# andrew-sha/CUDAFluidSimulator

Measured on AMD Instinct MI355X. Metric: particle-steps/sec (first 41 of the 100 steps of -m time), higher is better.
Workload: dtype f32

## Files before the change

### cudafluidsimulator_amd/csrc/sweeps_list.hip

```cpp
#include "sweep_common.h"

#define SL_NONE 0xFFFFFFFFu

#ifndef SL_WINDOW
#define SL_WINDOW 160
#endif
#ifndef SL_K1_THREADS
#define SL_K1_THREADS 64
#endif

#ifndef SL_K1_WAVES
#define SL_K1_WAVES 6
#endif
__device__ __forceinline__ void sl_store_quiet(const SweepArgs &A, int i, bool valid, float rho, int lane) {
    const unsigned long long calm = A.calm[(i - lane) >> 6];
    const float prs = fmaxf(0.f, SPH_GAS_CONSTANT * (rho - SPH_REST_DENSITY));
    const bool q = valid && prs == 0.f && ((calm >> lane) & 1ull);
    const unsigned long long qb = __ballot(q), vb = __ballot(valid);
    if (lane == 0) {
        reinterpret_cast<unsigned long long *>(A.quiet)[(i - lane) >> 6] = qb;
        if (A.quietAll && qb != vb) *A.quietAll = 0u;
    }
}
__device__ __forceinline__ uint32_t sl_quiet_window(const uint32_t *__restrict__ quiet, uint32_t j) {
    const uint32_t lo = quiet[j >> 5], hi = quiet[(j >> 5) + 1];
    return __builtin_amdgcn_alignbit(hi, lo, j & 31u);
}

template <bool FAST, bool SAMECUT>
__global__ __launch_bounds__(SL_K1_THREADS, SL_K1_WAVES * SL_K1_THREADS / 64)
void k_density_mask_lds(DevParams P, SweepArgs A) {
    __shared__ float4 stageAll[SL_K1_THREADS / SPH_WAVE][SW_CAP + SW_UNROLL];
    const int lane = threadIdx.x & 63, w = threadIdx.x >> 6;
    float4 *stage = stageAll[w];
    const int wv = xcd_tile(blockIdx.x, gridDim.x, A.tileChunk * (256 / SL_K1_THREADS), A.tileRotate) * (SL_K1_THREADS / SPH_WAVE) + w;
    const int i = A.i_origin + wv * SPH_WAVE + lane;
    const bool valid = i >= A.i_begin && i < A.i_end;
    const bool anyValid = __ballot(valid) != 0ull;
    float4 pi = valid ? A.pos4[i] : make_float4(0, 0, 0, 0);
    int3 c = sweep_cell(P, pi.x, pi.y, pi.z);
    int js[9], je[9];
    load_runs(P, A.cellRange, c, valid, js, je);

    int words = 0;
    uint32_t pairs = 0;
#pragma unroll
    for (int r = 0; r < 9; ++r) {
        words += (je[r] - js[r] + 31) >> 5;
        pairs += (uint32_t)(je[r] - js[r]);
    }
    const int Q = __builtin_amdgcn_readfirstlane((wave_max_i32(words) + 1) >> 1);
    const int shard = wv & (SL_POOL_SHARDS - 1);
    unsigned long long base = 0;
    if (lane == 0) base = atomicAdd(A.maskCursor + shard * SL_CURSOR_STRIDE, (unsigned long long)Q * SPH_WAVE);
    base = (unsigned long long)__builtin_amdgcn_readfirstlane((unsigned)(base >> 32)) << 32 |
           (unsigned long long)__builtin_amdgcn_readfirstlane((unsigned)base);
    const unsigned long long subCap = A.maskCapacity / SL_POOL_SHARDS;
    const bool ok = base + (unsigned long long)Q * SPH_WAVE <= subCap;
    base += (unsigned long long)shard * subCap;
    if (lane == 0 && anyValid) {
        A.maskOff[2 * (size_t)wv] = ok ? (uint32_t)base : SL_NONE;
        A.maskOff[2 * (size_t)wv + 1] = (uint32_t)Q;
        if (!ok) A.noneList[atomicAdd(A.maskCursor + 1, 1ull)] = (uint32_t)wv;
    }
    uint4 *const myq = reinterpret_cast<uint4 *>(A.maskPool) + (ok ? base : 0ull) + lane;
    if (A.pairCounter) {
        uint32_t s = wave_sum_u32(pairs);
        if (lane == 0) atomicAdd(A.pairCounter + 16 + (wv & 255) * 16, (unsigned long long)s);
    }

    if (lane < SW_UNROLL) stage[SW_CAP + lane] = make_float4(1e18f, 1e18f, 1e18f, 0.f);
    const float4 *const sent = stage + SW_CAP;
    float rho = 0.f;
    float h2v = P.h2, dcv = P.dcoef, cut2r = P.cut2, massv = SPH_MASS;
    asm volatile("" : "+v"(h2v), "+v"(dcv), "+v"(cut2r), "+v"(massv));
    uint32_t pj0 = 0, pm0 = 0;
    bool pending = false;
    int qidx = 0;
    uint32_t hcount = 0;
    auto emit = [&](uint32_t jbase, uint32_t mask) {
        if (ok && mask != 0) {
            hcount += (uint32_t)__builtin_popcount(mask);
            if (!pending) {
                pj0 = jbase;
                pm0 = mask;
                pending = true;
            } else {
                myq[(size_t)qidx * SPH_WAVE] = make_uint4(pj0, pm0, jbase, mask);
                ++qidx;
                pending = false;
            }
        }
    };
    const int rowId = c.y + c.z * P.D;
    unsigned long long todo = __ballot(valid);
    bool unify = false;
    if (todo) {
        const int row0 = __builtin_amdgcn_readlane(rowId, __ffsll((long long)todo) - 1);
        if (__ballot(valid && rowId != row0)) {
            unify = true;
#pragma unroll
            for (int r = 0; r < 9; ++r) {
                const unsigned long long mm = __ballot(valid && je[r] > js[r]);
                if (mm) {
                    const int u0 = __builtin_amdgcn_readlane(js[r], __ffsll((long long)mm) - 1);
                    const int u1 = __builtin_amdgcn_readlane(je[r], 63 - __clzll((long long)mm));
                    unify = unify && (u1 - u0) <= SW_CAP;
                }
            }
        }
    }
    struct Run {
        int jsr, len, u0, ulen;
        bool any, staged;
    };
    auto describe = [&](int r, bool act) -> Run {
        int jsr = js[0], jer = je[0];
#pragma unroll
        for (int q = 1; q < 9; ++q) {
            jsr = (r == q) ? js[q] : jsr;
            jer = (r == q) ? je[q] : jer;
        }
        Run R;
        const bool nonempty = act && jer > jsr;
        const unsigned long long mm = __ballot(nonempty);
        R.any = mm != 0;
        const int lo = mm ? __ffsll((long long)mm) - 1 : 0;
        const int hi = mm ? 63 - __clzll((long long)mm) : 0;
        R.u0 = __builtin_amdgcn_readlane(jsr, lo);
        R.ulen = R.any ? __builtin_amdgcn_readlane(jer, hi) - R.u0 : 0;
        R.staged = R.ulen <= SW_CAP;
        R.jsr = nonempty ? jsr : R.u0;
        R.len = nonempty ? jer - jsr : 0;
        return R;
    };
    while (todo) {
        const int leader = __ffsll((long long)todo) - 1;
        const int rowL = __builtin_amdgcn_readlane(rowId, leader);
        const bool act = valid && (unify || rowId == rowL);
        todo &= ~__ballot(act);
#pragma unroll 1
        for (int r = 0; r < 9; ++r) {
            const Run R = describe(r, act);
            if (R.any && R.staged) {
                for (int k = lane; k < R.ulen; k += SPH_WAVE) stage[k] = A.pos4[R.u0 + k];
                __builtin_amdgcn_fence(__ATOMIC_RELEASE, "wavefront");
                __builtin_amdgcn_wave_barrier();
            }
            if (R.any) {
                const int jsr = R.jsr, len = R.len;
                const float4 *cur = stage + (jsr - R.u0);
                const float4 *gcur = A.pos4 + jsr;
                uint32_t m = 0;
                int k = 0;
                auto trip = [&](const float4 (&pj)[SW_UNROLL]) {
#pragma unroll
                    for (int u = 0; u < SW_UNROLL; ++u) {
                        float dx = pi.x - pj[u].x;
                        float dy = pi.y - pj[u].y;
                        float dz = pi.z - pj[u].z;
                        float dist2;
                        float draw;
                        if (FAST) {
                            dist2 = __builtin_fmaf(dz, dz, __builtin_fmaf(dy, dy, dx * dx));
                            draw = h2v - dist2;
                            const float diff = fmaxf(draw, 0.f);
                            rho = __builtin_fmaf((massv * dcv) * (diff * diff), diff, rho);
                        } else {
                            dist2 = dx * dx + dy * dy + dz * dz;
                            draw = h2v - dist2;
                            float diff;
                            asm("v_max_f32_e32 %0, 0, %1" : "=v"(diff) : "v"(draw));
                            rho += massv * (dcv * diff * diff * diff);
                        }
                        if (SAMECUT) {
                            m = __builtin_amdgcn_alignbit(m, __float_as_uint(draw), 31);
                            continue;
                        }
                        asm("v_cmp_ngt_f32_e32 vcc, %1, %2\n\tv_addc_co_u32_e32 %0, vcc, %0, %0, vcc"
                            : "+v"(m)
                            : "v"(dist2), "v"(cut2r)
                            : "vcc");
                    }
#pragma unroll
                    for (int u = 0; u < SW_UNROLL; ++u) asm volatile("" ::"v"(pj[u].w));
                    if (((k + SW_UNROLL) & 31) == 0) {
                        if (SAMECUT) emit((uint32_t)(jsr + (k & ~31)), ~__builtin_bitreverse32(m));
                        else emit((uint32_t)(jsr + (k & ~31)), __builtin_bitreverse32(m));
                        m = 0;
                    }
                };
                if (R.staged) {
                    for (; __ballot(k < len); k += SW_UNROLL) {
                        float4 pj[SW_UNROLL];
#pragma unroll
                        for (int u = 0; u < SW_UNROLL; ++u) {
                            const float4 *p = (k + u < len) ? cur + k : sent;
                            pj[u] = p[u];
                        }
                        trip(pj);
                    }
                } else {
                    for (; __ballot(k < len); k += SW_UNROLL) {
                        float4 pj[SW_UNROLL];
#pragma unroll
                        for (int u = 0; u < SW_UNROLL; ++u) {
                            const bool in = k + u < len;
                            pj[u] = gcur[in ? k + u : 0];
                            pj[u].x = in ? pj[u].x : 1e18f;
                        }
                        trip(pj);
                    }
                }
                if ((k & 31) != 0) {
                    if (SAMECUT) emit((uint32_t)(jsr + (k & ~31)), (~__builtin_bitreverse32(m)) >> (32 - (k & 31)));
                    else emit((uint32_t)(jsr + (k & ~31)), __builtin_bitreverse32(m) >> (32 - (k & 31)));
                }
                __builtin_amdgcn_fence(__ATOMIC_ACQUIRE, "wavefront");
                __builtin_amdgcn_wave_barrier();
            }
        }
    }
    if (ok && valid) {
        if (pending) myq[(size_t)qidx * SPH_WAVE] = make_uint4(pj0, pm0, 0u, 0u);
        else if (qidx < Q) myq[(size_t)qidx * SPH_WAVE] = make_uint4(0u, 0u, 0u, 0u);
    }
    if (valid) {
        rho = fmaxf(rho, SPH_EPS_F);
        if (A.rhoToVel4) A.vel4[i].w = rho;
        A.pv8[2 * (size_t)i + 1].w = rho;
    }
    if (A.quiet) sl_store_quiet(A, i, valid, rho, lane);
    if (A.hitCount && valid) A.hitCount[i] = hcount;
}

#ifndef SL_SORT_SHIFT
#define SL_SORT_SHIFT 3
#endif
#define SL_DEAL_THREADS 256
#define SL_DEAL_ROWS SL_DEAL_THREADS
#define SL_DEAL_WINDOW (SL_DEAL_ROWS + SL_WINDOW - SPH_WAVE)
static_assert(SL_WINDOW >= SPH_WAVE, "the dealt sweep needs the window");

template <bool FAST, bool SLIM>
__global__ __launch_bounds__(SL_DEAL_THREADS) void k_force_dealt(DevParams P, SweepArgs A) {
    __shared__ uint32_t sortBase[128];
    __shared__ uint16_t rowOf[SL_DEAL_ROWS];
    __shared__ float4 win[2 * SL_DEAL_WINDOW];
    const int t = threadIdx.x, lane = t & 63;
    const bool second = (int)blockIdx.x >= A.nblk1;
    const int rb = second ? A.i_begin2 : A.i_begin, re = second ? A.i_end2 : A.i_end;
    const int chunk = A.tileChunk > 0 ? max(A.tileChunk * 256 / SL_DEAL_ROWS, 1) : 0;
    const int group = ((rb - A.i_origin) >> 6) / (SL_DEAL_ROWS / SPH_WAVE) +
                      xcd_tile(second ? (int)blockIdx.x - A.nblk1 : (int)blockIdx.x,
                               second ? (int)gridDim.x - A.nblk1 : A.nblk1, chunk, A.tileRotate);
    const int R0 = A.i_origin + group * SL_DEAL_ROWS;
    const unsigned long long *const quiet64 = reinterpret_cast<const unsigned long long *>(A.quiet);

    unsigned long long qw = 0ull;
    bool inPlace = false;
    if (A.quiet) {
        const int r0 = R0 + (t & ~63);
        const int lo = max(rb - r0, 0), hi = min(re - r0, 64);
        const unsigned long long vm = hi > lo ? ((hi - lo == 64 ? ~0ull : (1ull << (hi - lo)) - 1ull) << lo) : 0ull;
        if (vm) qw = quiet64[r0 >> 6];
        inPlace = __syncthreads_and((qw & vm) == vm) != 0;
    }
    if (!inPlace) {
        for (int b = t; b < 128; b += SL_DEAL_THREADS) sortBase[b] = 0u;
        __syncthreads();
        const int row = R0 + t;
        const bool counted = row >= rb && row < re && !((qw >> lane) & 1ull);
        const uint32_t bucket = min((counted ? A.hitCount[row] : 0u) >> SL_SORT_SHIFT, 127u);
        const uint32_t slot = atomicAdd(&sortBase[bucket], 1u);
        __syncthreads();
        if (t < SPH_WAVE) {
            const uint32_t a = sortBase[2 * t], b = sortBase[2 * t + 1];
            uint32_t incl = a + b;
#pragma unroll
            for (int off = 1; off < SPH_WAVE; off <<= 1) {
                const uint32_t up = __shfl_up(incl, off);
                incl += t >= off ? up : 0u;
            }
            const uint32_t excl = incl - (a + b);
            sortBase[2 * t] = excl;
            sortBase[2 * t + 1] = excl + a;
        }
        __syncthreads();
        rowOf[sortBase[bucket] + slot] = (uint16_t)t;
    }

    const bool allQuiet = A.quietAll && __builtin_amdgcn_readfirstlane(*A.quietAll) != 0u &&
                          (!A.quietHalo || __builtin_amdgcn_readfirstlane(*A.quietHalo) != 0u);
    const int w0 = max(R0 - (SL_WINDOW - SPH_WAVE) / 2, 0);
    int wlen = max(min(SL_DEAL_WINDOW, A.n_all - w0), 0);
    {
        bool wanted = !allQuiet && wlen > 0;
        if (wanted && A.quiet) {
            const int k0 = w0 >> 6, k1 = (w0 + wlen - 1) >> 6;
            wanted = k0 + t <= k1 && quiet64[k0 + t] != ~0ull;
        }
        if (__syncthreads_or(wanted)) {
            for (int k = t; k < 2 * wlen; k += SL_DEAL_THREADS) win[k] = A.pv8[2 * (size_t)w0 + k];
            __syncthreads();
        } else {
            wlen = 0;
        }
    }

    {
        const int i = R0 + (inPlace ? t : (int)rowOf[t]);
        const bool inRange = i >= rb && i < re;
        const int iSafe = inRange ? i : rb;
        float4 pi = A.pv8[2 * (size_t)iSafe];
        const float4 vi = A.pv8[2 * (size_t)iSafe + 1];
        const float prs_i = fmaxf(0.f, SPH_GAS_CONSTANT * (vi.w - SPH_REST_DENSITY));
        const int rel = iSafe - A.i_origin;
        const uint32_t baseq = inRange ? A.maskOff[2 * (size_t)(rel >> 6)] : SL_NONE;
        const int Q = inRange ? (int)A.maskOff[2 * (size_t)(rel >> 6) + 1] : 0;
        const bool valid = inRange && baseq != SL_NONE;
        ForceAcc F = {0.f, 0.f, 0.f};
        if (!allQuiet) {
            const uint4 *const sbase = reinterpret_cast<const uint4 *>(A.maskPool);
            const uint32_t send = valid ? baseq + (uint32_t)Q * SPH_WAVE : 0u;
            uint32_t sidx = valid ? baseq + (uint32_t)(rel & 63) : 0u;
            uint32_t m = 0, mq[2] = {0u, 0u};
            int jb = 0, jq[2] = {0, 0};
            bool live = true;
            const bool qi = A.quiet && valid && ((A.quiet[i >> 5] >> (i & 31)) & 1u);
            auto fetch = [&]() {
                while (sidx < send) {
                    uint4 q = sbase[sidx];
                    sidx = (q.w == 0u) ? send : sidx + SPH_WAVE;
                    if (qi) {
                        q.y &= ~sl_quiet_window(A.quiet, q.x);
                        q.w &= ~sl_quiet_window(A.quiet, q.z);
                    }
                    if (q.y == 0u) {
                        q.x = q.z;
                        q.y = q.w;
                        q.w = 0u;
                    }
                    jq[0] = (int)q.x;
                    mq[0] = q.y;
                    jq[1] = (int)q.z;
                    mq[1] = q.w;
                    if (q.y != 0u) break;
                }
            };
            fetch();
            if (__ballot(mq[0] != 0u)) {
                auto pop = [&]() -> int {
                    if (m == 0) {
                        m = mq[0];
                        jb = jq[0];
                        mq[0] = mq[1];
                        jq[0] = jq[1];
                        mq[1] = 0;
                        if (mq[0] == 0) fetch();
                    }
                    live = (m | mq[0]) != 0;
                    const bool has = m != 0;
                    const int b = has ? __builtin_ctz(m) : 0;
                    m &= m - 1u;
                    return has ? jb + b : iSafe;
                };
                auto body = [&](const float4 &pj, const float4 &vj) {
                    if (FAST) force_pair_fast(P, pi.x, pi.y, pi.z, vi.x, vi.y, vi.z, prs_i, pj, vj, F);
                    else force_pair<SLIM>(P, pi.x, pi.y, pi.z, vi.x, vi.y, vi.z, prs_i, pj, vj, F);
                };
#define SD_UNDEF4(q) asm volatile("" : "=v"(q.x), "=v"(q.y), "=v"(q.z), "=v"(q.w));
#define SD_FETCH(j, p, v)                                                      \
    SD_UNDEF4(p)                                                               \
    SD_UNDEF4(v)                                                               \
    if ((unsigned)((j)-w0) >= (unsigned)wlen) {                                \
        p = A.pv8[2 * (size_t)(j)];                                            \
        v = A.pv8[2 * (size_t)(j) + 1];                                        \
    }
#define SD_USE(j, p, v)                                                        \
    if ((unsigned)((j)-w0) < (unsigned)wlen) {                                 \
        p = win[2 * ((j)-w0)];                                                 \
        v = win[2 * ((j)-w0) + 1];                                             \
    }                                                                          \
    body(p, v);
                float4 p0 = make_float4(0, 0, 0, 0), v0 = p0, p1 = p0, v1 = p0;
                int j0 = pop();
                SD_FETCH(j0, p0, v0)
                int j1 = pop();
                SD_FETCH(j1, p1, v1)
                for (;;) {
                    SD_USE(j0, p0, v0)
                    if (!__ballot(live)) { SD_USE(j1, p1, v1) break; }
                    j0 = pop();
                    SD_FETCH(j0, p0, v0)
                    SD_USE(j1, p1, v1)
                    if (!__ballot(live)) { SD_USE(j0, p0, v0) break; }
                    j1 = pop();
                    SD_FETCH(j1, p1, v1)
                }
#undef SD_FETCH
#undef SD_USE
#undef SD_UNDEF4
            }
        }
        if (valid) {
            float vx = vi.x, vy = vi.y, vz = vi.z;
            integrate_particle(P, pi, vx, vy, vz, F, vi.w);
            store_particle(A, i, pi, vx, vy, vz, vi.w, F);
        }
    }
}

__global__ __launch_bounds__(256) void k_halo_quiet(const float4 *__restrict__ pv8, int lo_end, int hi_begin, int n_all,
                                                    const float4 *__restrict__ vref, const uint32_t *__restrict__ ownedQuiet,
                                                    uint32_t *__restrict__ haloQuiet) {
    if (*ownedQuiet == 0u) return;
    const int t = blockIdx.x * blockDim.x + threadIdx.x;
    if (t >= lo_end + (n_all - hi_begin)) return;
    const int j = t < lo_end ? t : hi_begin + (t - lo_end);
    const float4 v = pv8[2 * (size_t)j + 1], r = *vref;
    const float prs = fmaxf(0.f, SPH_GAS_CONSTANT * (v.w - SPH_REST_DENSITY));
    if (!(prs == 0.f && v.x == r.x && v.y == r.y && v.z == r.z)) *haloQuiet = 0u;
}
void sph_launch_halo_quiet(const float4 *pv8, int lo_end, int hi_begin, int n_all, const float4 *vref,
                           const uint32_t *ownedQuiet, uint32_t *haloQuiet, hipStream_t s) {
    const int rows = lo_end + (n_all - hi_begin);
    if (rows > 0) k_halo_quiet<<<(rows + 255) / 256, 256, 0, s>>>(pv8, lo_end, hi_begin, n_all, vref, ownedQuiet, haloQuiet);
}

__global__ __launch_bounds__(256) void k_count_hits(SweepArgs A) {
    const int i = A.i_begin + blockIdx.x * blockDim.x + threadIdx.x;
    uint32_t n = 0, dropped = 0;
    if (i < A.i_end) {
        const int rel = i - A.i_origin, wv = rel >> 6;
        const uint32_t baseq = A.maskOff[2 * (size_t)wv];
        const int Q = (int)A.maskOff[2 * (size_t)wv + 1];
        if (baseq != SL_NONE) {
            const uint4 *q4 = reinterpret_cast<const uint4 *>(A.maskPool) + baseq + (rel & 63);
            const bool qi = A.quiet && ((A.quiet[i >> 5] >> (i & 31)) & 1u);
            for (int q = 0; q < Q; ++q) {
                const uint4 t = q4[(size_t)q * SPH_WAVE];
                n += (uint32_t)__builtin_popcount(t.y) + (uint32_t)__builtin_popcount(t.w);
                if (qi)
                    dropped += (uint32_t)__builtin_popcount(t.y & sl_quiet_window(A.quiet, t.x)) +
                               (uint32_t)__builtin_popcount(t.w & sl_quiet_window(A.quiet, t.z));
                if (t.w == 0u) break;
            }
        }
    }
    n = wave_sum_u32(n);
    dropped = wave_sum_u32(dropped);
    if ((threadIdx.x & 63) == 0 && n) {
        atomicAdd(A.pairCounter + 16 + (blockIdx.x & 255) * 16 + 15, (unsigned long long)n);
        atomicAdd(A.pairCounter + 16 + (blockIdx.x & 255) * 16 + 14, (unsigned long long)(n - dropped));
    }
}

void sph_launch_density_list(const DevParams &P, const SweepArgs &A, int mathMode, hipStream_t s) {
    int cnt = A.i_end - A.i_begin;
    if (cnt <= 0) return;
    int blocks = (A.i_end - A.i_origin + SL_K1_THREADS - 1) / SL_K1_THREADS;
    const bool same = P.cut2 == P.h2;
    if (mathMode == 1) {
        if (same) k_density_mask_lds<true, true><<<blocks, SL_K1_THREADS, 0, s>>>(P, A);
        else k_density_mask_lds<true, false><<<blocks, SL_K1_THREADS, 0, s>>>(P, A);
    } else {
        if (same) k_density_mask_lds<false, true><<<blocks, SL_K1_THREADS, 0, s>>>(P, A);
        else k_density_mask_lds<false, false><<<blocks, SL_K1_THREADS, 0, s>>>(P, A);
    }
    if (A.pairCounter) k_count_hits<<<(cnt + 255) / 256, 256, 0, s>>>(A);
}

#define SL_FALLBACK_BLOCKS 512
template <bool FAST, bool SLIM>
__global__ __launch_bounds__(SPH_WAVE) void k_force_fallback(DevParams P, SweepArgs A) {
    const unsigned count = (unsigned)A.maskCursor[1];
    for (unsigned idx = blockIdx.x; idx < count; idx += gridDim.x) {
    const int i = A.i_origin + (int)A.noneList[idx] * SPH_WAVE + (int)threadIdx.x;
    const bool mine = (i >= A.i_begin && i < A.i_end) || (i >= A.i_begin2 && i < A.i_end2);
    if (!__ballot(mine)) continue;
    const int iSafe = mine ? i : A.i_begin;
    float4 pi = A.pv8[2 * (size_t)iSafe];
    const float4 vi = A.pv8[2 * (size_t)iSafe + 1];
    const float prs_i = fmaxf(0.f, SPH_GAS_CONSTANT * (vi.w - SPH_REST_DENSITY));
    int3 c = sweep_cell(P, pi.x, pi.y, pi.z);
    int js[9], je[9];
    load_runs(P, A.cellRange, c, mine, js, je);
    ForceAcc F = {0.f, 0.f, 0.f};
#pragma unroll
    for (int r = 0; r < 9; ++r)
        for (int j = js[r]; j < je[r]; ++j) {
            if (FAST) force_pair_fast(P, pi.x, pi.y, pi.z, vi.x, vi.y, vi.z, prs_i, A.pv8[2 * (size_t)j], A.pv8[2 * (size_t)j + 1], F);
            else force_pair<SLIM>(P, pi.x, pi.y, pi.z, vi.x, vi.y, vi.z, prs_i, A.pv8[2 * (size_t)j], A.pv8[2 * (size_t)j + 1], F);
        }
    if (mine) {
        float vx = vi.x, vy = vi.y, vz = vi.z;
        integrate_particle(P, pi, vx, vy, vz, F, vi.w);
        store_particle(A, i, pi, vx, vy, vz, vi.w, F);
    }
    }
}

__global__ void k_patch_pv8(const float4 *__restrict__ vel4, float4 *__restrict__ pv8, int i_begin,
                            int i_end, int n_all) {
    int t = blockIdx.x * blockDim.x + threadIdx.x;
    int j = t < i_begin ? t : i_end + (t - i_begin);
    if (j < n_all) pv8[2 * (size_t)j + 1] = vel4[j];
}

void sph_launch_patch_halo(const SweepArgs &A, hipStream_t s) {
    const int halo = A.i_begin + (A.n_all - A.i_end);
    if (halo > 0) k_patch_pv8<<<(halo + 255) / 256, 256, 0, s>>>(A.vel4, A.pv8, A.i_begin, A.i_end, A.n_all);
}

void sph_launch_force_list(const DevParams &P, const SweepArgs &A, int mathMode, hipStream_t s) {
    SweepArgs B = A;
    if (B.i_end2 <= B.i_begin2) B.i_begin2 = B.i_end2 = 0;
    if (B.i_end <= B.i_begin) {
        B.i_begin = B.i_begin2;
        B.i_end = B.i_end2;
        B.i_begin2 = B.i_end2 = 0;
    }
    if (B.i_end <= B.i_begin) return;
    if (B.patchHalo) sph_launch_patch_halo(B, s);
    const int wpb = SL_DEAL_ROWS / SPH_WAVE, threads = SL_DEAL_THREADS;
    auto blocks_of = [&](int a, int b) {
        if (b <= a) return 0;
        const int w0 = (a - B.i_origin) >> 6, w1 = (b - B.i_origin + 63) >> 6;
        return (w1 + wpb - 1) / wpb - w0 / wpb;
    };
    B.nblk1 = blocks_of(B.i_begin, B.i_end);
    const int fblocks = B.nblk1 + blocks_of(B.i_begin2, B.i_end2);
    const int blocks = SL_FALLBACK_BLOCKS;
    if (mathMode == 1) {
        k_force_dealt<true, true><<<fblocks, threads, 0, s>>>(P, B);
        k_force_fallback<true, true><<<blocks, SPH_WAVE, 0, s>>>(P, B);
    } else if (P.slimDiv) {
        k_force_dealt<false, true><<<fblocks, threads, 0, s>>>(P, B);
        k_force_fallback<false, true><<<blocks, SPH_WAVE, 0, s>>>(P, B);
    } else {
        k_force_dealt<false, false><<<fblocks, threads, 0, s>>>(P, B);
        k_force_fallback<false, false><<<blocks, SPH_WAVE, 0, s>>>(P, B);
    }
}
```

Baseline: 4.432 billion.

## Software-pipeline global neighbor loads in density kernel's unstaged path

For neighbor runs too large to stage in LDS, the density kernel now prefetches the next group of neighbor positions into registers while computing on the current group. Each slot is refilled right after use, and sched_barrier keeps the loads issued in place. Load indices are clamped so no out-of-range conditional select is needed on the address, and a 32-bit byte-offset addressing variant is used unless the particle count is huge. This hides global-memory latency in the unstaged loop, at the cost of extra register pressure, redundant loads past the run end, and more template instantiations.

```diff
diff --git a/cudafluidsimulator_amd/csrc/sweeps_list.hip b/cudafluidsimulator_amd/csrc/sweeps_list.hip
--- a/cudafluidsimulator_amd/csrc/sweeps_list.hip
+++ b/cudafluidsimulator_amd/csrc/sweeps_list.hip
@@ -27,7 +27,7 @@
     return __builtin_amdgcn_alignbit(hi, lo, j & 31u);
 }
 
-template <bool FAST, bool SAMECUT>
+template <bool FAST, bool SAMECUT, bool WIDE>
 __global__ __launch_bounds__(SL_K1_THREADS, SL_K1_WAVES * SL_K1_THREADS / 64)
 void k_density_mask_lds(DevParams P, SweepArgs A) {
     __shared__ float4 stageAll[SL_K1_THREADS / SPH_WAVE][SW_CAP + SW_UNROLL];
@@ -150,12 +150,17 @@
             if (R.any) {
                 const int jsr = R.jsr, len = R.len;
                 const float4 *cur = stage + (jsr - R.u0);
-                const float4 *gcur = A.pos4 + jsr;
                 uint32_t m = 0;
                 int k = 0;
-                auto trip = [&](const float4 (&pj)[SW_UNROLL]) {
+                auto noRefill = [](int) {};
+                auto trip = [&](auto fromGlobal, float4 (&pj)[SW_UNROLL], auto refill) {
+                    constexpr bool ROTATE = !std::is_same<decltype(refill), decltype(noRefill)>::value;
 #pragma unroll
                     for (int u = 0; u < SW_UNROLL; ++u) {
+                        if (decltype(fromGlobal)::value) {
+                            asm("" : "+v"(pj[u].x));
+                            pj[u].x = (k + u < len) ? pj[u].x : 1e18f;
+                        }
                         float dx = pi.x - pj[u].x;
                         float dy = pi.y - pj[u].y;
                         float dz = pi.z - pj[u].z;
@@ -175,42 +180,49 @@
                         }
                         if (SAMECUT) {
                             m = __builtin_amdgcn_alignbit(m, __float_as_uint(draw), 31);
-                            continue;
+                        } else {
+                            asm("v_cmp_ngt_f32_e32 vcc, %1, %2\n\tv_addc_co_u32_e32 %0, vcc, %0, %0, vcc"
+                                : "+v"(m)
+                                : "v"(dist2), "v"(cut2r)
+                                : "vcc");
                         }
-                        asm("v_cmp_ngt_f32_e32 vcc, %1, %2\n\tv_addc_co_u32_e32 %0, vcc, %0, %0, vcc"
-                            : "+v"(m)
-                            : "v"(dist2), "v"(cut2r)
-                            : "vcc");
-                    }
-#pragma unroll
-                    for (int u = 0; u < SW_UNROLL; ++u) asm volatile("" ::"v"(pj[u].w));
+                        if (ROTATE) {
+                            asm volatile("" ::"v"(pj[u].w));
+                            refill(u);
+                        }
+                    }
+                    if (!ROTATE) {
+#pragma unroll
+                        for (int u = 0; u < SW_UNROLL; ++u) asm volatile("" ::"v"(pj[u].w));
+                    }
                     if (((k + SW_UNROLL) & 31) == 0) {
                         if (SAMECUT) emit((uint32_t)(jsr + (k & ~31)), ~__builtin_bitreverse32(m));
                         else emit((uint32_t)(jsr + (k & ~31)), __builtin_bitreverse32(m));
                         m = 0;
                     }
                 };
+                float4 pj[SW_UNROLL];
                 if (R.staged) {
                     for (; __ballot(k < len); k += SW_UNROLL) {
-                        float4 pj[SW_UNROLL];
 #pragma unroll
                         for (int u = 0; u < SW_UNROLL; ++u) {
                             const float4 *p = (k + u < len) ? cur + k : sent;
                             pj[u] = p[u];
                         }
-                        trip(pj);
+                        trip(std::false_type(), pj, noRefill);
                     }
                 } else {
-                    for (; __ballot(k < len); k += SW_UNROLL) {
-                        float4 pj[SW_UNROLL];
-#pragma unroll
-                        for (int u = 0; u < SW_UNROLL; ++u) {
-                            const bool in = k + u < len;
-                            pj[u] = gcur[in ? k + u : 0];
-                            pj[u].x = in ? pj[u].x : 1e18f;
-                        }
-                        trip(pj);
-                    }
+                    const int last = max(len - 1, 0);
+                    auto load = [&](int kk, int u) {
+                        const uint32_t j = (uint32_t)(jsr + min(kk + u, last));
+                        if (WIDE) pj[u] = A.pos4[(size_t)j];
+                        else pj[u] = *reinterpret_cast<const float4 *>(reinterpret_cast<const char *>(A.pos4) + (j << 4));
+                        __builtin_amdgcn_sched_barrier(0);
+                    };
+#pragma unroll
+                    for (int u = 0; u < SW_UNROLL; ++u) load(0, u);
+                    for (; __ballot(k < len); k += SW_UNROLL)
+                        trip(std::true_type(), pj, [&](int u) { load(k + SW_UNROLL, u); });
                 }
                 if ((k & 31) != 0) {
                     if (SAMECUT) emit((uint32_t)(jsr + (k & ~31)), (~__builtin_bitreverse32(m)) >> (32 - (k & 31)));
@@ -461,13 +473,18 @@
     if (cnt <= 0) return;
     int blocks = (A.i_end - A.i_origin + SL_K1_THREADS - 1) / SL_K1_THREADS;
     const bool same = P.cut2 == P.h2;
+    const bool wide = A.n_all > (1 << 28);
+#define SL_LAUNCH(F, C)                                                                    \
+    (wide ? k_density_mask_lds<F, C, true><<<blocks, SL_K1_THREADS, 0, s>>>(P, A)       \
+          : k_density_mask_lds<F, C, false><<<blocks, SL_K1_THREADS, 0, s>>>(P, A))
     if (mathMode == 1) {
-        if (same) k_density_mask_lds<true, true><<<blocks, SL_K1_THREADS, 0, s>>>(P, A);
-        else k_density_mask_lds<true, false><<<blocks, SL_K1_THREADS, 0, s>>>(P, A);
+        if (same) SL_LAUNCH(true, true);
+        else SL_LAUNCH(true, false);
     } else {
-        if (same) k_density_mask_lds<false, true><<<blocks, SL_K1_THREADS, 0, s>>>(P, A);
-        else k_density_mask_lds<false, false><<<blocks, SL_K1_THREADS, 0, s>>>(P, A);
-    }
+        if (same) SL_LAUNCH(false, true);
+        else SL_LAUNCH(false, false);
+    }
+#undef SL_LAUNCH
     if (A.pairCounter) k_count_hits<<<(cnt + 255) / 256, 256, 0, s>>>(A);
 }
 
```

New measurement: 4.457 billion, median of 2. About the same (+0.6%).
